# chenjiaoAngel/Paddle-Lite

Measured on AMD Instinct MI355X. Metric: INT8 images/sec MobileNetV1 224x224, higher is better.
Workload: dtype int8; 1 GPU; MobileNetV1 INT8 full graph 224x224 (27 int8 convs + pool + fc + softmax), random-init weights, 128 images per step and GPU (4 predictors / HIP streams, each running whole steps: 4 steps in flight), input resident in HBM; steps_in_flight=4, global_batch=128

## Files before the change

paddle-lite_amd/csrc/fused_dwpw_i8.hip:

```cpp
#include <stdlib.h>

#include <type_traits>

#include "plhip_device.h"
#include "plhip_kernels.h"
#include "dw_common.h"
#include "gemm_tr_common.h"

namespace plhip {

constexpr int FW_TR = 7;
constexpr int FW_NT = 4;

constexpr int FW_STAMP_SLOTS = 16;

template <int DELTA>
__device__ __forceinline__ void fw_load_row(const int8_t* __restrict__ xs, uint32_t off, uint32_t (&d)[2]) {
  __builtin_memcpy(d, xs + off + DELTA, 8);
}

template <int MTW, int OUT, bool DWNN, bool PWNN>
__global__ __launch_bounds__(512, 2) void fused_dwpw14_kernel(FusedArgs a) {
  const GemmArgs& g = a.pw;
  PLHIP_PRELOAD(a.x); PLHIP_PRELOAD(a.dw_w); PLHIP_PRELOAD(a.dw_scale); PLHIP_PRELOAD(a.dw_bias); PLHIP_PRELOAD(a.dw_act);
  PLHIP_PRELOAD(a.dw_alpha); PLHIP_PRELOAD(a.n); PLHIP_PRELOAD(a.C); PLHIP_PRELOAD(a.tiles); PLHIP_PRELOAD(a.ones); PLHIP_PRELOAD(g.wp); PLHIP_PRELOAD(g.y);
  PLHIP_PRELOAD(g.scale); PLHIP_PRELOAD(g.bias); PLHIP_PRELOAD(g.M); PLHIP_PRELOAD(g.KS); PLHIP_PRELOAD(g.act); PLHIP_PRELOAD(g.alpha);
  extern __shared__ __attribute__((aligned(16))) uint8_t fw_lds[];
  const int lane = threadIdx.x & 63;
  const int wave = __builtin_amdgcn_readfirstlane(threadIdx.x >> 6);
  const unsigned nb = (unsigned)a.tiles, per = (nb + 7) >> 3;
  const unsigned vb = (blockIdx.x & 7) * per + (blockIdx.x >> 3);
  if (vb >= nb) return;
  const int b = (int)(vb >> 1), hf = (int)(vb & 1);
  unsigned long long* const gstamp = PLHIP_STAMPS_OF(g);
  const bool diag = kStamps && gstamp && vb < 1024;
  unsigned long long* const lstamp = diag ? gstamp + ((size_t)vb * 8 + wave) * FW_STAMP_SLOTS : nullptr;
  PLHIP_STAMP_REAL(0);
  PLHIP_STAMP(1);
  const int KS = g.KS, C = a.C, R = KS >> 2;
  const int c = lane & 31, h = lane >> 5;

  const int chl = lane >> 2, q = lane & 3;
  const uint32_t sel_lo = q == 0 ? 0x0201000cu : (q == 1 ? 0x03020100u : (q == 2 ? 0x04030201u : 0x0c070605u));
  const uint32_t sel_hi = q == 0 ? 0x06050403u : (q == 1 ? 0x07060504u : (q == 2 ? 0x0c070605u : 0x0c0c0c0cu));
  uint32_t xoff = (uint32_t)(((b * C + 16 * wave + chl) * 14 + 7 * hf) * 14 + (q == 0 ? 0 : (q == 1 ? 3 : 6)));
  const uint32_t top = hf == 0 ? 0u : 0xffffffffu, bot = hf == 1 ? 0u : 0xffffffffu;
  const int8_t* const xs0 = a.x + (hf == 0 ? 0 : -14);
  const int8_t* const xs8 = a.x + (hf == 1 ? 84 : 98);
  const int ch0 = 16 * wave + chl;
  uint32_t wbase = (uint32_t)((ch0 >> 5) * FW_KSTEP + ((ch0 >> 3) & 3) * 1024 + (ch0 & 7) * 128 + ((ch0 & 6) << 4) + 4 * q);
  const float dw_hi2 = a.dw_act == ACT_RELU6 ? fminf(a.dw_alpha + a.dw_alpha, 254.f) : 254.f;
  const float dw_leak = a.dw_act == ACT_LEAKY ? a.dw_alpha : 1.f;

  uint32_t in[9][2];
  uint32_t wr[3];
  float dsc, dbi;
  auto load_row = [&](auto t_c, uint32_t off, uint32_t (&d)[2]) __attribute__((always_inline)) {
    constexpr int t = decltype(t_c)::value;
    if constexpr (t == 0) fw_load_row<0>(xs0, off, d);
    else if constexpr (t == 8) fw_load_row<0>(xs8, off, d);
    else fw_load_row<14 * (t - 1)>(a.x, off, d);
  };
  auto fetch_task = [&](int ch, uint32_t off) __attribute__((always_inline)) {
    const int8_t* wp = a.dw_w + (size_t)ch * 9;
    uint32_t w0, w1, w2;
    __builtin_memcpy(&w0, wp, 4);
    __builtin_memcpy(&w1, wp + 3, 4);
    __builtin_memcpy(&w2, wp + 5, 4);
    wr[0] = w0 & 0xffffffu;
    wr[1] = w1 & 0xffffffu;
    wr[2] = w2 >> 8;
    const float s = a.dw_scale[ch], bb = a.dw_bias ? a.dw_bias[ch] : 0.f;
    dsc = s + s;
    dbi = bb + bb;
    load_row(std::integral_constant<int, 0>{}, off, in[0]);
    load_row(std::integral_constant<int, 1>{}, off, in[1]);
    load_row(std::integral_constant<int, 2>{}, off, in[2]);
    load_row(std::integral_constant<int, 3>{}, off, in[3]);
    load_row(std::integral_constant<int, 4>{}, off, in[4]);
    load_row(std::integral_constant<int, 5>{}, off, in[5]);
    load_row(std::integral_constant<int, 6>{}, off, in[6]);
    load_row(std::integral_constant<int, 7>{}, off, in[7]);
    load_row(std::integral_constant<int, 8>{}, off, in[8]);
  };

  uint32_t tr00;
  {
    const int qr = (lane & 15) >> 1, par = (lane >> 4) & 1;
    tr00 = (uint32_t)((h * 2) * 1024 + qr * 128 + ((2 * (qr >> 1) + par) * 16) + (lane & 1) * 8);
  }
  const int mt0 = wave * MTW;
  const uint8_t* const wpk = reinterpret_cast<const uint8_t*>(g.wp) + (size_t)mt0 * KS * 1024;
  const uint32_t wlane = (uint32_t)lane * 16;
  v4i W[4][MTW];
  auto fetch_w = [&](int j, int ks) __attribute__((always_inline)) {
#pragma unroll
    for (int m = 0; m < MTW; ++m) W[j][m] = *reinterpret_cast<const v4i*>(wpk + ((size_t)m * KS + ks) * 1024 + wlane);
  };
  v16i acc[FW_NT][MTW];
#pragma unroll
  for (int n = 0; n < FW_NT; ++n)
#pragma unroll
    for (int m = 0; m < MTW; ++m)
#pragma unroll
      for (int r = 0; r < 16; ++r) acc[n][m][r] = 0;

  using std::integral_constant;
  auto round = [&](auto produce_c, auto consume_c, int rp, int rc) __attribute__((always_inline)) {
    constexpr bool PRODUCE = decltype(produce_c)::value, CONSUME = decltype(consume_c)::value;
    const int rn = rp + 1 < R ? rp + 1 : rp;
    const int nch = 128 * rn + 16 * wave + chl;
    const uint32_t noff = xoff + (uint32_t)(rn - rp) * (128 * 196);
    const uint32_t wb = wbase + (uint32_t)rp * (4 * FW_KSTEP);
    const uint32_t rb = (uint32_t)rc * (4 * FW_KSTEP);
    int dacc[FW_TR][4];
    const uint32_t wr0t = wr[0] & top, wr2b = wr[2] & bot;
    uint32_t nwr[3];
    float ndsc = 0.f, ndbi = 0.f;
    v2i lo[FW_NT], hi[FW_NT];
    auto read_frag = [&](int j, int n) __attribute__((always_inline)) {
      const uint32_t ta = (tr00 + rb) ^ (uint32_t)(n << 5);
      lo[n] = __builtin_amdgcn_ds_read_tr8_b64_v2i32((lds_v2i_ptr_t)(fw_lds + ta + j * FW_KSTEP));
      hi[n] = __builtin_amdgcn_ds_read_tr8_b64_v2i32((lds_v2i_ptr_t)(fw_lds + ta + j * FW_KSTEP + 1024));
    };
    auto mfma = [&](auto i_c) __attribute__((always_inline)) {
      constexpr int i = decltype(i_c)::value;
      constexpr int j = i / (FW_NT * MTW), n = (i / MTW) % FW_NT, m = i % MTW;
      if constexpr (m == 0) {
        if constexpr (n == 0 && j == 0) {
          read_frag(0, 0);
          read_frag(0, 1);
        }
        constexpr int nn = (n + 2) % FW_NT, jn = j + (n + 2) / FW_NT;
        if constexpr (jn < 4) read_frag(jn, nn);
      }
      const v4i av = {lo[n][0], lo[n][1], hi[n][0], hi[n][1]};
      acc[n][m] = __builtin_amdgcn_mfma_i32_32x32x32_i8(av, W[j][m], acc[n][m], 0, 0, 0);
      if constexpr (n == FW_NT - 1 && m == MTW - 1) {
        const int ksn = 4 * (rc + 1) + j;
        fetch_w(j, ksn < KS ? ksn : KS - 1);
      }
    };
    auto mfmas = [&](auto self, auto i_c, auto end_c) __attribute__((always_inline)) -> void {
      constexpr int i = decltype(i_c)::value, end = decltype(end_c)::value;
      if constexpr (i < end) {
        mfma(integral_constant<int, i>{});
        self(self, integral_constant<int, i + 1>{}, integral_constant<int, end>{});
      }
    };
    constexpr int NM = 4 * FW_NT * MTW;
    constexpr auto mstart = [](int t) {
      constexpr int cum[10] = {0, 1, 3, 7, 11, 15, 19, 23, 28, 32};
      return cum[t] * NM / 32;
    };
    auto taps = [&](auto t_c) __attribute__((always_inline)) {
      constexpr int t = decltype(t_c)::value;
      const uint32_t e0 = __builtin_amdgcn_perm(in[t][1], in[t][0], sel_lo), e1 = __builtin_amdgcn_perm(in[t][1], in[t][0], sel_hi);
      uint32_t win[4];
      win[0] = e0;
      win[1] = __builtin_amdgcn_alignbyte(e1, e0, 1);
      win[2] = __builtin_amdgcn_alignbyte(e1, e0, 2);
      win[3] = __builtin_amdgcn_alignbyte(e1, e0, 3);
#pragma unroll
      for (int r = 0; r < 3; ++r) {
        const int o = t - r;
        if (o < 0 || o >= FW_TR) continue;
#pragma unroll
        for (int jj = 0; jj < 4; ++jj)
          dacc[o][jj] = r == 0 ? sdot4_first(win[jj], t == 0 ? wr0t : wr[0])
                               : __builtin_amdgcn_sdot4((int)win[jj], (int)(t == 8 ? wr2b : wr[r]), dacc[o][jj], false);
      }
      load_row(integral_constant<int, t>{}, noff, in[t]);
      if constexpr (t == 2) {
        const int8_t* wp = a.dw_w + (size_t)nch * 9;
        uint32_t w0, w1, w2;
        __builtin_memcpy(&w0, wp, 4);
        __builtin_memcpy(&w1, wp + 3, 4);
        __builtin_memcpy(&w2, wp + 5, 4);
        nwr[0] = w0 & 0xffffffu;
        nwr[1] = w1 & 0xffffffu;
        nwr[2] = w2 >> 8;
        ndsc = a.dw_scale[nch];
        ndbi = (a.dw_bias ? a.dw_bias : a.dw_scale)[nch];
        if (!a.dw_bias) ndbi = 0.f;
      }
    };
    auto finish = [&](auto o_c) __attribute__((always_inline)) {
      constexpr int o = decltype(o_c)::value;
      const uint32_t pk = DWNN ? requant4_nn_rtz(dacc[o], dsc, dbi, dw_hi2, a.ones) : dw_requant4<ACT_LEAKY>(dacc[o], dsc, dbi, dw_leak, -254.f, 254.f);
      *reinterpret_cast<uint32_t*>(fw_lds + (wb ^ (uint32_t)(o << 4))) = pk;
    };
    auto chunk = [&](auto t_c) __attribute__((always_inline)) {
      constexpr int t = decltype(t_c)::value;
      mfmas(mfmas, integral_constant<int, mstart(t)>{}, integral_constant<int, mstart(t + 1)>{});
      __builtin_amdgcn_sched_barrier(0);
    };
    constexpr auto m1start = [](int o) {
      constexpr int cum[8] = {0, 5, 10, 14, 19, 23, 28, 32};
      return cum[o] * NM / 32;
    };
    auto slice = [&](auto o_c) __attribute__((always_inline)) {
      constexpr int o = decltype(o_c)::value;
      if constexpr (CONSUME) mfmas(mfmas, integral_constant<int, m1start(o)>{}, integral_constant<int, m1start(o + 1)>{});
      finish(o_c);
      __builtin_amdgcn_sched_barrier(0);
    };
    if constexpr (!PRODUCE) {
      chunk(integral_constant<int, 0>{});
      chunk(integral_constant<int, 1>{});
      chunk(integral_constant<int, 2>{});
      chunk(integral_constant<int, 3>{});
      chunk(integral_constant<int, 4>{});
      chunk(integral_constant<int, 5>{});
      chunk(integral_constant<int, 6>{});
      chunk(integral_constant<int, 7>{});
      chunk(integral_constant<int, 8>{});
    } else {
      taps(integral_constant<int, 0>{});
      taps(integral_constant<int, 1>{});
      taps(integral_constant<int, 2>{});
      taps(integral_constant<int, 3>{});
      taps(integral_constant<int, 4>{});
      taps(integral_constant<int, 5>{});
      taps(integral_constant<int, 6>{});
      taps(integral_constant<int, 7>{});
      taps(integral_constant<int, 8>{});
      __builtin_amdgcn_sched_barrier(0);
      slice(integral_constant<int, 0>{});
      slice(integral_constant<int, 1>{});
      slice(integral_constant<int, 2>{});
      slice(integral_constant<int, 3>{});
      slice(integral_constant<int, 4>{});
      slice(integral_constant<int, 5>{});
      slice(integral_constant<int, 6>{});
    }
    if constexpr (PRODUCE) {
      wr[0] = nwr[0];
      wr[1] = nwr[1];
      wr[2] = nwr[2];
      dsc = ndsc + ndsc;
      dbi = ndbi + ndbi;
    }
  };

  fetch_task(ch0, xoff);
  fetch_w(0, 0);
  fetch_w(1, 1 < KS ? 1 : KS - 1);
  fetch_w(2, 2 < KS ? 2 : KS - 1);
  fetch_w(3, 3 < KS ? 3 : KS - 1);
  PLHIP_STAMP(2);
  round(std::true_type{}, std::false_type{}, 0, 0);
  xoff += (R > 1 ? 1 : 0) * 128 * 196;
  PLHIP_STAMP(3);
  __syncthreads();
  for (int r = 1; r < R; ++r) {
    round(std::true_type{}, std::true_type{}, r, r - 1);
    xoff += (r + 1 < R ? 1 : 0) * 128 * 196;
    if (r < 5) PLHIP_STAMP(4 + 2 * (r - 1));
    __syncthreads();
    if (r < 5) PLHIP_STAMP(5 + 2 * (r - 1));
  }
  float psc[MTW], pbi[MTW];
#pragma unroll
  for (int m = 0; m < MTW; ++m) {
    psc[m] = 1.f;
    pbi[m] = 0.f;
    if (OUT != OUT_I32) {
      psc[m] = g.scale[(mt0 + m) * 32 + c];
      if (g.bias) pbi[m] = g.bias[(mt0 + m) * 32 + c];
    }
  }
  const int orow0 = FW_TR * hf;
  if (OUT == OUT_I8) {
    const float hi2 = g.act == ACT_RELU6 ? fminf(g.alpha + g.alpha, 254.f) : 254.f;
    const float leak = g.act == ACT_LEAKY ? g.alpha : 1.f;
    uint8_t* stg = fw_lds + (size_t)KS * FW_KSTEP + wave * (32 * MTW * FW_SP);
    const uint32_t rbf = (uint32_t)(R - 1) * (4 * FW_KSTEP);
    v2i flo[2][4], fhi[2][4];
    auto read_tile = [&](auto n_c) __attribute__((always_inline)) {
      constexpr int n = decltype(n_c)::value;
      const uint32_t ta = (tr00 + rbf) ^ (uint32_t)(n << 5);
#pragma unroll
      for (int j = 0; j < 4; ++j) {
        flo[n & 1][j] = __builtin_amdgcn_ds_read_tr8_b64_v2i32((lds_v2i_ptr_t)(fw_lds + ta + j * FW_KSTEP));
        fhi[n & 1][j] = __builtin_amdgcn_ds_read_tr8_b64_v2i32((lds_v2i_ptr_t)(fw_lds + ta + j * FW_KSTEP + 1024));
      }
    };
    auto mfma_tile = [&](auto n_c) __attribute__((always_inline)) {
      constexpr int n = decltype(n_c)::value;
#pragma unroll
      for (int j = 0; j < 4; ++j) {
        const v4i av = {flo[n & 1][j][0], flo[n & 1][j][1], fhi[n & 1][j][0], fhi[n & 1][j][1]};
#pragma unroll
        for (int m = 0; m < MTW; ++m) acc[n][m] = __builtin_amdgcn_mfma_i32_32x32x32_i8(av, W[j][m], acc[n][m], 0, 0, 0);
      }
    };
    auto epi_tile = [&](auto n_c) __attribute__((always_inline)) {
      constexpr int n = decltype(n_c)::value;
#pragma unroll
      for (int m = 0; m < MTW; ++m) {
        const float s2 = psc[m] + psc[m], b2 = pbi[m] + pbi[m];
        uint32_t edw[4] = {0, 0, 0, 0};
#pragma unroll
        for (int gq = 0; gq < 4; ++gq) {
          if (n == FW_NT - 1 && gq >= 2) continue;
          int v[4] = {acc[n][m][4 * gq], acc[n][m][4 * gq + 1], acc[n][m][4 * gq + 2], acc[n][m][4 * gq + 3]};
          edw[gq] = PWNN ? requant4_nn_rtz(v, s2, b2, hi2, a.ones) : dw_requant4<ACT_LEAKY>(v, s2, b2, leak, -254.f, 254.f);
        }
        auto s02 = __builtin_amdgcn_permlane32_swap(edw[0], edw[2], false, false);
        auto s13 = __builtin_amdgcn_permlane32_swap(edw[1], edw[3], false, false);
        const uint32_t d0 = s02[0], d1 = s02[1], d2 = s13[0], d3 = s13[1];
        if (n < FW_NT - 1 || h == 0) {
          uint16_t* p = reinterpret_cast<uint16_t*>(stg + (32 * m + c) * FW_SP + (2 * n + h) * 14);
          p[0] = (uint16_t)d0; p[1] = (uint16_t)(d0 >> 16);
          p[2] = (uint16_t)d1; p[3] = (uint16_t)(d1 >> 16);
          p[4] = (uint16_t)d2; p[5] = (uint16_t)(d2 >> 16);
          p[6] = (uint16_t)d3;
        }
      }
    };
    using I0 = integral_constant<int, 0>;
    using I1 = integral_constant<int, 1>;
    using I2 = integral_constant<int, 2>;
    using I3 = integral_constant<int, 3>;
    read_tile(I0{});
    read_tile(I1{});
    mfma_tile(I0{});
    __builtin_amdgcn_sched_barrier(0);
    read_tile(I2{});
    mfma_tile(I1{});
    epi_tile(I0{});
    __builtin_amdgcn_sched_barrier(0);
    read_tile(I3{});
    mfma_tile(I2{});
    epi_tile(I1{});
    __builtin_amdgcn_sched_barrier(0);
    mfma_tile(I3{});
    epi_tile(I2{});
    __builtin_amdgcn_sched_barrier(0);
    PLHIP_STAMP(12);
    epi_tile(I3{});
    PLHIP_STAMP(13);
    const int piece = lane & 7, rsub = lane >> 3;
    int8_t* ybase = reinterpret_cast<int8_t*>(g.y) + ((size_t)b * g.M + mt0 * 32) * 196 + 98 * hf + piece * 16;
#pragma unroll
    for (int i = 0; i < 4 * MTW; ++i) {
      const int row = 8 * i + rsub;
      const v4i v = *reinterpret_cast<const v4i*>(stg + row * FW_SP + (piece < 7 ? piece : 6) * 16);
      int8_t* yp = ybase + (size_t)row * 196;
      if (piece < 6) __builtin_memcpy(yp, &v, 16);
      else if (piece == 6) {
        const uint16_t t2 = (uint16_t)v[0];
        __builtin_memcpy(yp, &t2, 2);
      }
    }
  } else {
    round(std::false_type{}, std::true_type{}, R, R - 1);
    PLHIP_STAMP(12);
    const float fcap = g.act == ACT_RELU6 ? g.alpha : __builtin_huge_valf();
    const float flo = (g.act == ACT_RELU || g.act == ACT_RELU6) ? 0.f : -__builtin_huge_valf();
#pragma unroll
    for (int m = 0; m < MTW; ++m) {
      const size_t chan = ((size_t)b * g.M + (mt0 + m) * 32 + c) * 196;
#pragma unroll
      for (int n = 0; n < FW_NT; ++n) {
#pragma unroll
        for (int gq = 0; gq < 4; ++gq) {
          const int o = 2 * n + (gq >> 1);
          if (o >= FW_TR) continue;
          const int col = 8 * (gq & 1) + 4 * h;
          const size_t off = chan + (size_t)(orow0 + o) * 14 + col;
          if (OUT == OUT_F32) {
            float f[4];
#pragma unroll
            for (int e = 0; e < 4; ++e) {
              float y = __fmaf_rn((float)acc[n][m][4 * gq + e], psc[m], pbi[m]);
              if (g.act == ACT_LEAKY) y = y > 0.f ? y : g.alpha * y;
              f[e] = fminf(fmaxf(y, flo), fcap);
            }
            float* yp = reinterpret_cast<float*>(g.y) + off;
            if (col + 3 < 14) {
              const v4f v = {f[0], f[1], f[2], f[3]};
              __builtin_memcpy(yp, &v, 16);
            } else if (col < 14) {
              yp[0] = f[0];
              yp[1] = f[1];
            }
          } else {
            int* yp = reinterpret_cast<int*>(g.y) + off;
            if (col + 3 < 14) {
              const v4i v = {acc[n][m][4 * gq], acc[n][m][4 * gq + 1], acc[n][m][4 * gq + 2], acc[n][m][4 * gq + 3]};
              __builtin_memcpy(yp, &v, 16);
            } else if (col < 14) {
              yp[0] = acc[n][m][4 * gq];
              yp[1] = acc[n][m][4 * gq + 1];
            }
          }
        }
      }
    }
  }
  PLHIP_STAMP(14);
  if (diag) {
    asm volatile("s_waitcnt vmcnt(0)" ::: "memory");
    PLHIP_STAMP(15);
  }
}

void launch_fused_dwpw(const FusedArgs& a_in, const DwPlan& p, int out, hipStream_t s) {
  FusedArgs a = a_in;
  a.tiles = p.tiles;
  a.pw.NT = p.NT;
  a.ones = 0x01010101u;
  if (p.family == DWPW_7) return run_fused_small(p, a, out, s);
  if (p.family == DWPW_STREAM) return run_fused_stream(p, a, out, s);
  PLHIP_SET_STAMPS(a.pw, "fw", sizeof(unsigned long long) * 1024 * 8 * FW_STAMP_SLOTS);
  with_const<1, 2>(p.MTW, [&](auto mtw) {
    with_out_nonneg<OUT_I32, OUT_F32, OUT_I8>(out, a.dw_act, a.pw.act, [&](auto out_c, auto dn, auto pn) {
      constexpr int OUT = decltype(out_c)::value;
      constexpr bool DN = decltype(dn)::value != 0, PN = decltype(pn)::value != 0;
      if constexpr (OUT == OUT_I8 || !PN) launch_max_lds(fused_dwpw14_kernel<decltype(mtw)::value, OUT, DN, PN>, p, s, a);
    });
  });
}

}
```

Measured before the change: 417,400 img/s.

## Stage depthwise input rows through LDS and specialize fused dw-pw kernel on K rounds

```diff
diff --git a/paddle-lite_amd/csrc/fused_dwpw_i8.hip b/paddle-lite_amd/csrc/fused_dwpw_i8.hip
--- a/paddle-lite_amd/csrc/fused_dwpw_i8.hip
+++ b/paddle-lite_amd/csrc/fused_dwpw_i8.hip
@@ -11,6 +11,10 @@
 
 constexpr int FW_TR = 7;
 constexpr int FW_NT = 4;
+constexpr int FW_RP = 20;
+constexpr int FW_CP = 208;
+constexpr int FW_STAGE_AT = 5;
+static_assert(16 * FW_CP <= 32 * FW_SP && 16 * FW_CP % 16 == 0, "the row stage lives in one wave's staging slice of the M = 256 form");
 
 constexpr int FW_STAMP_SLOTS = 16;
 
@@ -19,8 +23,8 @@
   __builtin_memcpy(d, xs + off + DELTA, 8);
 }
 
-template <int MTW, int OUT, bool DWNN, bool PWNN>
-__global__ __launch_bounds__(512, 2) void fused_dwpw14_kernel(FusedArgs a) {
+template <int MTW, int OUT, bool DWNN, bool PWNN, int R>
+__device__ __forceinline__ void fused_dwpw14_body(const FusedArgs& a) {
   const GemmArgs& g = a.pw;
   PLHIP_PRELOAD(a.x); PLHIP_PRELOAD(a.dw_w); PLHIP_PRELOAD(a.dw_scale); PLHIP_PRELOAD(a.dw_bias); PLHIP_PRELOAD(a.dw_act);
   PLHIP_PRELOAD(a.dw_alpha); PLHIP_PRELOAD(a.n); PLHIP_PRELOAD(a.C); PLHIP_PRELOAD(a.tiles); PLHIP_PRELOAD(a.ones); PLHIP_PRELOAD(g.wp); PLHIP_PRELOAD(g.y);
@@ -37,13 +41,20 @@
   unsigned long long* const lstamp = diag ? gstamp + ((size_t)vb * 8 + wave) * FW_STAMP_SLOTS : nullptr;
   PLHIP_STAMP_REAL(0);
   PLHIP_STAMP(1);
-  const int KS = g.KS, C = a.C, R = KS >> 2;
+  constexpr int KS = 4 * R;
+  const int C = a.C;
   const int c = lane & 31, h = lane >> 5;
 
   const int chl = lane >> 2, q = lane & 3;
   const uint32_t sel_lo = q == 0 ? 0x0201000cu : (q == 1 ? 0x03020100u : (q == 2 ? 0x04030201u : 0x0c070605u));
   const uint32_t sel_hi = q == 0 ? 0x06050403u : (q == 1 ? 0x07060504u : (q == 2 ? 0x0c070605u : 0x0c0c0c0cu));
-  uint32_t xoff = (uint32_t)(((b * C + 16 * wave + chl) * 14 + 7 * hf) * 14 + (q == 0 ? 0 : (q == 1 ? 3 : 6)));
+  constexpr bool STAGED = OUT == OUT_I8;
+  const uint32_t stage0 = (uint32_t)(KS * FW_KSTEP + wave * (32 * MTW * FW_SP));
+  const uint32_t rdb = stage0 + (uint32_t)(chl * FW_CP + 4 * q);
+  const uint32_t wst = stage0 + (uint32_t)((lane >> 3) * FW_CP + ((lane & 7) + 1 - hf) * FW_RP);
+  const uint32_t xrow = (uint32_t)(((b * C + 16 * wave + (lane >> 3)) * 14 + 6 * hf + (lane & 7)) * 14);
+  const uint32_t nb1 = STAGED && xrow + (uint32_t)(8 * 196 + (R - 1) * (128 * 196) + 15) > (uint32_t)(a.n * C * 196) ? 1u : 0u;
+  uint32_t xoff = STAGED ? xrow - 1u - nb1 : (uint32_t)(((b * C + 16 * wave + chl) * 14 + 7 * hf) * 14 + (q == 0 ? 0 : (q == 1 ? 3 : 6)));
   const uint32_t top = hf == 0 ? 0u : 0xffffffffu, bot = hf == 1 ? 0u : 0xffffffffu;
   const int8_t* const xs0 = a.x + (hf == 0 ? 0 : -14);
   const int8_t* const xs8 = a.x + (hf == 1 ? 84 : 98);
@@ -83,6 +94,35 @@
     load_row(std::integral_constant<int, 7>{}, off, in[7]);
     load_row(std::integral_constant<int, 8>{}, off, in[8]);
   };
+  v4i nx[2];
+  auto load_rows = [&](uint32_t off) __attribute__((always_inline)) {
+    __builtin_memcpy(&nx[0], a.x + off, 16);
+    __builtin_memcpy(&nx[1], a.x + off + 8 * 196, 16);
+  };
+  auto fetch_params = [&](int ch, uint32_t (&w)[3], float& s, float& bb) __attribute__((always_inline)) {
+    const int8_t* wp = a.dw_w + (size_t)ch * 9;
+    uint32_t w0, w1, w2;
+    __builtin_memcpy(&w0, wp, 4);
+    __builtin_memcpy(&w1, wp + 3, 4);
+    __builtin_memcpy(&w2, wp + 5, 4);
+    w[0] = w0 & 0xffffffu;
+    w[1] = w1 & 0xffffffu;
+    w[2] = w2 >> 8;
+    s = a.dw_scale[ch];
+    bb = (a.dw_bias ? a.dw_bias : a.dw_scale)[ch];
+    if (!a.dw_bias) bb = 0.f;
+  };
+  auto stage_rows = [&]() __attribute__((always_inline)) {
+#pragma unroll
+    for (int i = 0; i < 2; ++i) {
+      const uint32_t d0 = (uint32_t)nx[i][0], d1 = (uint32_t)nx[i][1], d2 = (uint32_t)nx[i][2], d3 = (uint32_t)nx[i][3];
+      uint32_t* p = reinterpret_cast<uint32_t*>(fw_lds + wst + i * (8 * FW_CP));
+      p[0] = __builtin_amdgcn_alignbyte(d1, d0, nb1) & 0xffffff00u;
+      p[1] = __builtin_amdgcn_alignbyte(d2, d1, nb1);
+      p[2] = __builtin_amdgcn_alignbyte(d3, d2, nb1);
+      p[3] = __builtin_amdgcn_alignbyte(0u, d3, nb1) & 0x00ffffffu;
+    }
+  };
 
   uint32_t tr00;
   {
@@ -98,23 +138,20 @@
     for (int m = 0; m < MTW; ++m) W[j][m] = *reinterpret_cast<const v4i*>(wpk + ((size_t)m * KS + ks) * 1024 + wlane);
   };
   v16i acc[FW_NT][MTW];
-#pragma unroll
-  for (int n = 0; n < FW_NT; ++n)
-#pragma unroll
-    for (int m = 0; m < MTW; ++m)
-#pragma unroll
-      for (int r = 0; r < 16; ++r) acc[n][m][r] = 0;
+  const v16i zero16 = {0, 0, 0, 0, 0, 0, 0, 0, 0, 0, 0, 0, 0, 0, 0, 0};
 
   using std::integral_constant;
-  auto round = [&](auto produce_c, auto consume_c, int rp, int rc) __attribute__((always_inline)) {
+  auto round = [&](auto produce_c, auto consume_c, auto first_c, auto last_c, int rp, int rc) __attribute__((always_inline)) {
     constexpr bool PRODUCE = decltype(produce_c)::value, CONSUME = decltype(consume_c)::value;
-    const int rn = rp + 1 < R ? rp + 1 : rp;
-    const int nch = 128 * rn + 16 * wave + chl;
-    const uint32_t noff = xoff + (uint32_t)(rn - rp) * (128 * 196);
+    constexpr bool FIRST = decltype(first_c)::value, LAST = decltype(last_c)::value;
+    constexpr bool NEXT_TASK = PRODUCE && !LAST;
+    constexpr bool NEXT_W = PRODUCE;
+    const int nch = 128 * (rp + 1) + 16 * wave + chl;
+    const uint32_t noff = xoff + (uint32_t)(128 * 196);
     const uint32_t wb = wbase + (uint32_t)rp * (4 * FW_KSTEP);
     const uint32_t rb = (uint32_t)rc * (4 * FW_KSTEP);
     int dacc[FW_TR][4];
-    const uint32_t wr0t = wr[0] & top, wr2b = wr[2] & bot;
+    const uint32_t wr0t = STAGED ? wr[0] : wr[0] & top, wr2b = STAGED ? wr[2] : wr[2] & bot;
     uint32_t nwr[3];
     float ndsc = 0.f, ndbi = 0.f;
     v2i lo[FW_NT], hi[FW_NT];
@@ -135,11 +172,8 @@
         if constexpr (jn < 4) read_frag(jn, nn);
       }
       const v4i av = {lo[n][0], lo[n][1], hi[n][0], hi[n][1]};
-      acc[n][m] = __builtin_amdgcn_mfma_i32_32x32x32_i8(av, W[j][m], acc[n][m], 0, 0, 0);
-      if constexpr (n == FW_NT - 1 && m == MTW - 1) {
-        const int ksn = 4 * (rc + 1) + j;
-        fetch_w(j, ksn < KS ? ksn : KS - 1);
-      }
+      acc[n][m] = __builtin_amdgcn_mfma_i32_32x32x32_i8(av, W[j][m], FIRST && j == 0 ? zero16 : acc[n][m], 0, 0, 0);
+      if constexpr (NEXT_W && n == FW_NT - 1 && m == MTW - 1) fetch_w(j, 4 * (rc + 1) + j);
     };
     auto mfmas = [&](auto self, auto i_c, auto end_c) __attribute__((always_inline)) -> void {
       constexpr int i = decltype(i_c)::value, end = decltype(end_c)::value;
@@ -155,7 +189,15 @@
     };
     auto taps = [&](auto t_c) __attribute__((always_inline)) {
       constexpr int t = decltype(t_c)::value;
-      const uint32_t e0 = __builtin_amdgcn_perm(in[t][1], in[t][0], sel_lo), e1 = __builtin_amdgcn_perm(in[t][1], in[t][0], sel_hi);
+      uint32_t e0, e1;
+      if constexpr (STAGED) {
+        const uint32_t* rp2 = reinterpret_cast<const uint32_t*>(fw_lds + rdb + t * FW_RP);
+        e0 = rp2[0];
+        e1 = rp2[1];
+      } else {
+        e0 = __builtin_amdgcn_perm(in[t][1], in[t][0], sel_lo);
+        e1 = __builtin_amdgcn_perm(in[t][1], in[t][0], sel_hi);
+      }
       uint32_t win[4];
       win[0] = e0;
       win[1] = __builtin_amdgcn_alignbyte(e1, e0, 1);
@@ -170,19 +212,10 @@
           dacc[o][jj] = r == 0 ? sdot4_first(win[jj], t == 0 ? wr0t : wr[0])
                                : __builtin_amdgcn_sdot4((int)win[jj], (int)(t == 8 ? wr2b : wr[r]), dacc[o][jj], false);
       }
-      load_row(integral_constant<int, t>{}, noff, in[t]);
-      if constexpr (t == 2) {
-        const int8_t* wp = a.dw_w + (size_t)nch * 9;
-        uint32_t w0, w1, w2;
-        __builtin_memcpy(&w0, wp, 4);
-        __builtin_memcpy(&w1, wp + 3, 4);
-        __builtin_memcpy(&w2, wp + 5, 4);
-        nwr[0] = w0 & 0xffffffu;
-        nwr[1] = w1 & 0xffffffu;
-        nwr[2] = w2 >> 8;
-        ndsc = a.dw_scale[nch];
-        ndbi = (a.dw_bias ? a.dw_bias : a.dw_scale)[nch];
-        if (!a.dw_bias) ndbi = 0.f;
+      if constexpr (NEXT_TASK) {
+        if constexpr (!STAGED) load_row(integral_constant<int, t>{}, noff, in[t]);
+        else if constexpr (t == FW_STAGE_AT) load_rows(noff);
+        if constexpr (t == 2) fetch_params(nch, nwr, ndsc, ndbi);
       }
     };
     auto finish = [&](auto o_c) __attribute__((always_inline)) {
@@ -232,9 +265,13 @@
       slice(integral_constant<int, 3>{});
       slice(integral_constant<int, 4>{});
       slice(integral_constant<int, 5>{});
+      if constexpr (STAGED && NEXT_TASK) {
+        stage_rows();
+        __builtin_amdgcn_sched_barrier(0);
+      }
       slice(integral_constant<int, 6>{});
     }
-    if constexpr (PRODUCE) {
+    if constexpr (NEXT_TASK) {
       wr[0] = nwr[0];
       wr[1] = nwr[1];
       wr[2] = nwr[2];
@@ -243,22 +280,65 @@
     }
   };
 
-  fetch_task(ch0, xoff);
+  if constexpr (STAGED) {
+    const v4i z4 = {0, 0, 0, 0};
+#pragma unroll
+    for (int i = 0; i < 4; ++i)
+      if (64 * i + lane < 16 * FW_CP / 16) *reinterpret_cast<v4i*>(fw_lds + stage0 + (64 * i + lane) * 16) = z4;
+    const bool first = xoff == 0xffffffffu;
+    load_rows(first ? 0u : xoff);
+    float s, bb;
+    fetch_params(ch0, wr, s, bb);
+    dsc = s + s;
+    dbi = bb + bb;
+    if (first) {
+#pragma unroll
+      for (int i = 0; i < 2; ++i) {
+        const uint32_t d0 = (uint32_t)nx[i][0], d1 = (uint32_t)nx[i][1], d2 = (uint32_t)nx[i][2], d3 = (uint32_t)nx[i][3];
+        nx[i][0] = (int)(d0 << 8);
+        nx[i][1] = (int)__builtin_amdgcn_alignbyte(d1, d0, 3);
+        nx[i][2] = (int)__builtin_amdgcn_alignbyte(d2, d1, 3);
+        nx[i][3] = (int)__builtin_amdgcn_alignbyte(d3, d2, 3);
+      }
+    }
+  } else {
+    fetch_task(ch0, xoff);
+  }
   fetch_w(0, 0);
-  fetch_w(1, 1 < KS ? 1 : KS - 1);
-  fetch_w(2, 2 < KS ? 2 : KS - 1);
-  fetch_w(3, 3 < KS ? 3 : KS - 1);
+  fetch_w(1, 1);
+  fetch_w(2, 2);
+  fetch_w(3, 3);
   PLHIP_STAMP(2);
-  round(std::true_type{}, std::false_type{}, 0, 0);
-  xoff += (R > 1 ? 1 : 0) * 128 * 196;
-  PLHIP_STAMP(3);
-  __syncthreads();
-  for (int r = 1; r < R; ++r) {
-    round(std::true_type{}, std::true_type{}, r, r - 1);
-    xoff += (r + 1 < R ? 1 : 0) * 128 * 196;
-    if (r < 5) PLHIP_STAMP(4 + 2 * (r - 1));
+  if constexpr (STAGED) stage_rows();
+  using T = std::true_type;
+  using F = std::false_type;
+  auto behind = [&](int r) __attribute__((always_inline)) {
+    if (r >= 1) {
+#pragma unroll
+      for (int n = 0; n < FW_NT; ++n)
+#pragma unroll
+        for (int m = 0; m < MTW; ++m) asm volatile("" : "+v"(acc[n][m]));
+    }
+    xoff += 128 * 196;
+    if (r == 0) PLHIP_STAMP(3);
+    else if (r < 5) PLHIP_STAMP(4 + 2 * (r - 1));
     __syncthreads();
-    if (r < 5) PLHIP_STAMP(5 + 2 * (r - 1));
+    if (r >= 1 && r < 5) PLHIP_STAMP(5 + 2 * (r - 1));
+  };
+  round(T{}, F{}, F{}, std::bool_constant<R == 1>{}, 0, 0);
+  behind(0);
+  if constexpr (R >= 2) {
+    round(T{}, T{}, T{}, std::bool_constant<R == 2>{}, 1, 0);
+    behind(1);
+  }
+  if constexpr (R >= 3) {
+    round(T{}, T{}, F{}, std::bool_constant<R == 3>{}, 2, 1);
+    behind(2);
+  }
+  if constexpr (R >= 4) {
+    static_assert(R <= 4, "C <= 512: dwpw_launch_plan");
+    round(T{}, T{}, F{}, T{}, 3, 2);
+    behind(3);
   }
   float psc[MTW], pbi[MTW];
 #pragma unroll
@@ -286,13 +366,14 @@
         fhi[n & 1][j] = __builtin_amdgcn_ds_read_tr8_b64_v2i32((lds_v2i_ptr_t)(fw_lds + ta + j * FW_KSTEP + 1024));
       }
     };
-    auto mfma_tile = [&](auto n_c) __attribute__((always_inline)) {
+    auto mfma_tile = [&](auto n_c, auto first_c) __attribute__((always_inline)) {
       constexpr int n = decltype(n_c)::value;
+      constexpr bool FIRST = decltype(first_c)::value;
 #pragma unroll
       for (int j = 0; j < 4; ++j) {
         const v4i av = {flo[n & 1][j][0], flo[n & 1][j][1], fhi[n & 1][j][0], fhi[n & 1][j][1]};
 #pragma unroll
-        for (int m = 0; m < MTW; ++m) acc[n][m] = __builtin_amdgcn_mfma_i32_32x32x32_i8(av, W[j][m], acc[n][m], 0, 0, 0);
+        for (int m = 0; m < MTW; ++m) acc[n][m] = __builtin_amdgcn_mfma_i32_32x32x32_i8(av, W[j][m], FIRST && j == 0 ? zero16 : acc[n][m], 0, 0, 0);
       }
     };
     auto epi_tile = [&](auto n_c) __attribute__((always_inline)) {
@@ -323,21 +404,24 @@
     using I1 = integral_constant<int, 1>;
     using I2 = integral_constant<int, 2>;
     using I3 = integral_constant<int, 3>;
-    read_tile(I0{});
-    read_tile(I1{});
-    mfma_tile(I0{});
-    __builtin_amdgcn_sched_barrier(0);
-    read_tile(I2{});
-    mfma_tile(I1{});
-    epi_tile(I0{});
-    __builtin_amdgcn_sched_barrier(0);
-    read_tile(I3{});
-    mfma_tile(I2{});
-    epi_tile(I1{});
-    __builtin_amdgcn_sched_barrier(0);
-    mfma_tile(I3{});
-    epi_tile(I2{});
-    __builtin_amdgcn_sched_barrier(0);
+    auto last_k_steps = [&](auto first_c) __attribute__((always_inline)) {
+      read_tile(I0{});
+      read_tile(I1{});
+      mfma_tile(I0{}, first_c);
+      __builtin_amdgcn_sched_barrier(0);
+      read_tile(I2{});
+      mfma_tile(I1{}, first_c);
+      epi_tile(I0{});
+      __builtin_amdgcn_sched_barrier(0);
+      read_tile(I3{});
+      mfma_tile(I2{}, first_c);
+      epi_tile(I1{});
+      __builtin_amdgcn_sched_barrier(0);
+      mfma_tile(I3{}, first_c);
+      epi_tile(I2{});
+      __builtin_amdgcn_sched_barrier(0);
+    };
+    last_k_steps(std::bool_constant<R == 1>{});
     PLHIP_STAMP(12);
     epi_tile(I3{});
     PLHIP_STAMP(13);
@@ -355,8 +439,11 @@
       }
     }
   } else {
-    round(std::false_type{}, std::true_type{}, R, R - 1);
+    round(F{}, T{}, std::bool_constant<R == 1>{}, T{}, R, R - 1);
     PLHIP_STAMP(12);
+    uint32_t tid = threadIdx.x;
+    asm volatile("" : "+v"(tid));
+    const int h = (int)(tid >> 5) & 1;
     const float fcap = g.act == ACT_RELU6 ? g.alpha : __builtin_huge_valf();
     const float flo = (g.act == ACT_RELU || g.act == ACT_RELU6) ? 0.f : -__builtin_huge_valf();
 #pragma unroll
@@ -407,6 +494,16 @@
   }
 }
 
+template <int MTW, int OUT, bool DWNN, bool PWNN>
+__global__ __launch_bounds__(512, 2) void fused_dwpw14_kernel(FusedArgs a) {
+  switch (a.pw.KS >> 2) {
+    case 1: return fused_dwpw14_body<MTW, OUT, DWNN, PWNN, 1>(a);
+    case 2: return fused_dwpw14_body<MTW, OUT, DWNN, PWNN, 2>(a);
+    case 3: return fused_dwpw14_body<MTW, OUT, DWNN, PWNN, 3>(a);
+    default: return fused_dwpw14_body<MTW, OUT, DWNN, PWNN, 4>(a);
+  }
+}
+
 void launch_fused_dwpw(const FusedArgs& a_in, const DwPlan& p, int out, hipStream_t s) {
   FusedArgs a = a_in;
   a.tiles = p.tiles;
```

Measured after the change: 434,600 img/s, median of 6. 1.04x the previous value.
